# indianajohn/akaze-rust

Measured on AMD Instinct MI355X. Metric: Mpix/s through extract_features (4 oct x 4 sub), higher is better.
Workload: dtype f32

## Files before the change

akaze-rust_amd/csrc/akz_api.cpp:

```cpp
#include <cstdio>

#include "akz_ctx.hpp"

unsigned akz::host_cpu_share() {
    unsigned n = std::max(1u, std::thread::hardware_concurrency());
    cpu_set_t set;
    if (sched_getaffinity(0, sizeof(set), &set) == 0) n = std::max(1, CPU_COUNT(&set));
    if (FILE* f = fopen("/sys/fs/cgroup/cpu.max", "r")) {
        char q[32] = {0};
        long period = 0;
        if (fscanf(f, "%31s %ld", q, &period) == 2 && period > 0 && strcmp(q, "max") != 0)
            n = std::min<unsigned>(n, (unsigned)std::max(1L, atol(q) / period));
        fclose(f);
    }
    if (const char* e = std::getenv("LOCAL_WORLD_SIZE")) {
        const int ranks = atoi(e);
        if (ranks > 1) n = std::max(2u, n / (unsigned)ranks);
    }
    return std::max(1u, n);
}

int level_info_out(const std::vector<LevelPlan>& plan, uint64_t level, double* etime, double* esigma,
                          uint32_t* octave, uint32_t* sublevel, uint32_t* sigma_size, uint32_t* lw, uint32_t* lh,
                          uint32_t* det_sigma, uint64_t* n_tau, double* tau, uint64_t tau_cap) {
// ... 283 lines not shown
                return AKZ_ERR_INVALID_ARG;
            }
    c->settings.host_threads = threads;
    push_settings(c);
    for (akz_ctx* x : all) x->workers.reset();
    return AKZ_OK;
}
int akz_ctx_set_candidate_hint(akz_ctx* c, uint32_t per_image) {
    AKZ_TRY(bind(c));
    c->cand_cap_hint = std::max<uint32_t>(per_image, 16u);
    for (akz_ctx* l : c->lanes) l->cand_cap_hint = c->cand_cap_hint.load();
    return AKZ_OK;
}
int akz_ctx_set_match_mode(akz_ctx* c, int mode) {
    AKZ_TRY(bind(c));
    if (mode < 0 || mode > 3) return AKZ_ERR_INVALID_ARG;
    c->settings.match_mode = mode;
    push_settings(c);
    return AKZ_OK;
}
int akz_ctx_set_fed_mode(akz_ctx* c, int mode) {
    AKZ_TRY(bind(c));
    if (mode != 0 && mode != 2) return AKZ_ERR_INVALID_ARG;
    c->settings.fed_mode = mode;
    push_settings(c);
    return AKZ_OK;
}
const char* akz_fed_kernel_name(void) { return "k_level_march + k_fed_own"; }
int akz_debug_march_bands(int kind, uint32_t w, uint32_t h, uint32_t n, int half_width, int32_t* rows, uint32_t cap,
                          uint32_t* n_bands) {
    if (!n_bands || (cap && !rows) || kind < 0 || kind > 1 || w < 16 || h < 16 || n == 0 || half_width < 1 || half_width > 4)
        return AKZ_ERR_INVALID_ARG;
    *n_bands = launch::march_band_rows(kind, w, h, n, half_width, rows, cap);
    return AKZ_OK;
}
int akz_debug_detector_set_cells(int half_width, const uint32_t* w, const uint32_t* h, uint32_t n_entries, uint32_t n, int32_t* cells,
                                 uint32_t cap, int32_t* grids, uint32_t* n_workgroups) {
    if (!n_workgroups || !w || !h || !grids || (cap && !cells) || n_entries < 1 || n_entries > launch::detector_march_set_max() || n == 0 ||
        half_width < 1 || half_width > 4)
        return AKZ_ERR_INVALID_ARG;
    for (uint32_t e = 0; e < n_entries; ++e)
        if (w[e] < 4u * (uint32_t)half_width + 8u || h[e] < 4u * (uint32_t)half_width + 8u) return AKZ_ERR_INVALID_ARG;
    *n_workgroups = launch::detector_set_cells(half_width, w, h, n_entries, n, cells, cap, grids);
    return AKZ_OK;
}
const char* akz_detector_kernel_name(void) { return "detector (k_detector_march + k_detector_tiled)"; }
int akz_debug_set_schedule(akz_ctx* c, int key, int value) {
    if (!c || key < 0 || key >= SCHED_COUNT_) return AKZ_ERR_INVALID_ARG;
    AKZ_TRY(bind(c));
    CtxSettings& s = c->settings;
    s.sched[key] = value;
    if (key == SCHED_DET_BAND_ROWS || key == SCHED_LEVEL_BAND_ROWS)
        launch::march_min_band_rows(s.sched[SCHED_DET_BAND_ROWS], s.sched[SCHED_LEVEL_BAND_ROWS]);
    if (key == SCHED_DET_SETS) launch::detector_set_waves(value >= 11 && value <= 14 ? value - 10 : 0);
    if (key == SCHED_JOB_KPX) {
        s.big_px_sync = value > 0 ? (uint64_t)value * 1000u : gates::kBigPxSync;
        s.big_px_async = value > 0 ? (uint64_t)value * 1000u : gates::kBigPxAsync;
        s.lane_px = value > 0 ? (uint64_t)value * 1000u : gates::kLanePx;
    }
    push_settings(c);
    return AKZ_OK;
}
int akz_debug_placement_verdict(float spin_pair_ms, float tiny_pair_ms, float tiny_alone_ms, float spin_ms) {
    return akz::placement_verdict(spin_pair_ms, tiny_pair_ms, tiny_alone_ms, spin_ms);
}
int akz_debug_stream_placement(akz_ctx* c, int* info) {
// ... 161 lines not shown
```

akaze-rust_amd/csrc/akz_internal.hpp:

```cpp
#pragma once
#include <hip/hip_runtime.h>

#include <cstdint>
#include <functional>
#include <string>
#include <vector>

#include "../../include/akaze_hip.h"
#include "../../include/akaze_hip_debug.h"

namespace akz {

void set_error(const std::string& msg);
unsigned host_cpu_share();

using TrialsOnDevice = std::function<int(const float*, const float*, const float*, const float*, uint32_t, const uint32_t*, uint32_t,
                                         float, float, float*, int32_t*)>;
int remove_outliers_impl(const akz_keypoint* keypoints_0, uint64_t n0, const akz_keypoint* keypoints_1, uint64_t n1,
                         const akz_match* matches, uint64_t n_matches, uint64_t num_trials, float epsilon_model,
                         float epsilon_inlier, akz_match* out, uint64_t* n_out, const TrialsOnDevice& trials_on_device);

#define AKZ_HIP_TRY(expr)                                                                          \
    do {                                                                                           \
        hipError_t _e = (expr);                                                                    \
// ... 136 lines not shown
void contrast_max(hipStream_t s, const float* blurred, uint32_t w, uint32_t h, uint32_t n,
                  unsigned long long* d_hmax_bits);
void contrast_hist(hipStream_t s, const float* blurred, uint32_t w, uint32_t h, uint32_t n,
                   const unsigned long long* d_hmax_bits, uint32_t nbins, uint32_t* d_hist);
void contrast_final(hipStream_t s, const unsigned long long* d_hmax_bits, const uint32_t* d_hist, uint32_t nbins,
                    double percentile, uint32_t n, double* d_k);
bool blur_fused_supported(uint32_t ntaps);
void blur_fused_f32(hipStream_t s, const float* in, float* out, uint32_t w, uint32_t h, uint32_t n, const float* k,
                    uint32_t ntaps);
void blur_fused_u8(hipStream_t s, const uint8_t* in, float* out, uint32_t w, uint32_t h, uint32_t n, const float* k,
                   uint32_t ntaps);
void prep_fused(hipStream_t s, const float* prev, bool half, float* lt_out, float* lsmooth, float* lflow, uint32_t w,
                uint32_t h, uint32_t pw, uint32_t ph, uint32_t n, const float* g3, const double* d_k, uint32_t k_pow);
bool detector_fused_supported(uint32_t sigma);
void detector_fused(hipStream_t s, const float* lsmooth, uint32_t sigma, float* lx, float* ly, float* lxx, float* lyy,
                    float* lxy, float* ldet_out, uint32_t w, uint32_t h, uint32_t n);
bool detector_tiled_fused_supported(uint32_t sigma);
struct DetLevelDesc {
    const float* lsmooth;
    float *lx, *ly, *lxx, *lyy, *lxy, *ldet;
    uint32_t w, h, level;
    float border_m;
};
uint32_t detector_tiled_set_max();
void detector_tiled_set(hipStream_t s, uint32_t sigma, const DetLevelDesc* levels, uint32_t nlevels, uint32_t n, float thr,
                        Candidate* d_cand, uint32_t cap, uint32_t* d_count);
void detector_tiled_fused(hipStream_t s, const float* lsmooth, uint32_t sigma, float* lx, float* ly, float* lxx,
                          float* lyy, float* lxy, float* ldet_out, uint32_t w, uint32_t h, uint32_t n, uint32_t level,
                          float thr, float border_m, Candidate* d_cand, uint32_t cap, uint32_t* d_count);
bool blur5_stream_supported(uint32_t w, uint32_t h, uint32_t ntaps, bool is_u8);
void blur5_stream_u8(hipStream_t s, const uint8_t* in, float* out, uint32_t w, uint32_t h, uint32_t n, const float* k);
void blur5_stream_f32(hipStream_t s, const float* in, float* out, uint32_t w, uint32_t h, uint32_t n, const float* k);
uint32_t march_band_rows(int kind, uint32_t w, uint32_t h, uint32_t n, int S, int32_t* cs_ce, uint32_t cap);
bool blur5_march_supported(uint32_t w, uint32_t h, uint32_t ntaps);
void blur5_march_u8(hipStream_t s, const uint8_t* in, float* out, uint32_t w, uint32_t h, uint32_t n, const float* k);
void blur5_march_f32(hipStream_t s, const float* in, float* out, uint32_t w, uint32_t h, uint32_t n, const float* k);
bool contrast_march_supported(uint32_t w, uint32_t h, uint32_t ntaps, uint32_t nbins);
void contrast_march(hipStream_t s, const float* in, uint32_t w, uint32_t h, uint32_t n, const float* g3,
                    unsigned long long* d_hmax_bits, uint32_t nbins, uint32_t* d_hist, double* d_thr);
void contrast_thresholds(hipStream_t s, const unsigned long long* d_hmax_bits, uint32_t nbins, uint32_t n, double* d_thr);
bool contrast_stream_supported(uint32_t w, uint32_t h, uint32_t ntaps, uint32_t nbins);
void contrast_stream(hipStream_t s, const float* in, uint32_t w, uint32_t h, uint32_t n, const float* g3,
                     unsigned long long* d_hmax_bits, uint32_t nbins, uint32_t* d_hist, double* d_thr);
bool prep_stream_supported(uint32_t w, uint32_t h);
void prep_stream(hipStream_t s, const float* prev, bool half, float* lt_out, float* lsmooth, float* lflow, uint32_t w,
                 uint32_t h, uint32_t pw, uint32_t ph, uint32_t n, const float* g3, const double* d_k, uint32_t k_pow);
bool detector_march_supported(uint32_t sigma, uint32_t w, uint32_t h, float border_m, bool nms);
void detector_march(hipStream_t s, const float* lsmooth, uint32_t sigma, float* lx, float* ly, float* lxx, float* lyy,
                    float* lxy, float* ldet_out, uint32_t w, uint32_t h, uint32_t n, uint32_t level, float thr,
                    float border_m, Candidate* d_cand, uint32_t cap, uint32_t* d_count);
uint32_t detector_march_set_max();
void detector_march_set(hipStream_t s, uint32_t sigma, const DetLevelDesc* levels, uint32_t nlevels, uint32_t n, float thr,
                        Candidate* d_cand, uint32_t cap, uint32_t* d_count);
void detector_set_waves(int waves);
uint32_t detector_set_cells(int S, const uint32_t* w, const uint32_t* h, uint32_t nlv, uint32_t n, int32_t* cells, uint32_t cap,
                            int32_t* grids);
bool head_fused_supported(uint32_t w, uint32_t h, uint32_t ntaps0, uint32_t ntaps1);
void head_fused_u8(hipStream_t s, const uint8_t* in, float* lt0, float* blurred, float* gx, float* gy, uint32_t w, uint32_t h, uint32_t n,
                   const float* k5, const float* g3, unsigned long long* d_smax_bits, uint32_t* d_zero_word = nullptr);
void head_fused_f32(hipStream_t s, const float* in, float* lt0, float* blurred, float* gx, float* gy, uint32_t w, uint32_t h, uint32_t n,
                    const float* k5, const float* g3, unsigned long long* d_smax_bits, uint32_t* d_zero_word = nullptr);
void contrast_hist_final(hipStream_t s, const float* gx, const float* gy, uint32_t w, uint32_t h, uint32_t n, unsigned long long* d_smax_bits,
                         uint32_t nbins, uint32_t* d_hist, uint32_t* d_done, double percentile, double* d_k);
void flow_from_pair(hipStream_t s, const float* gx, const float* gy, float* lflow, uint32_t w, uint32_t h, uint32_t n, const double* d_k,
                    uint32_t k_pow);
void march_min_band_rows(int detector, int level);
// ... 198 lines not shown
```

akaze-rust_amd/csrc/akz_march.hip:

```cpp
#include <hip/hip_runtime.h>

#include <algorithm>
#include <cstdlib>
#include <type_traits>

#include "akz_internal.hpp"
#include "akz_pm_g2.hpp"

namespace akz {
namespace {

typedef float f2 __attribute__((ext_vector_type(2)));
typedef float f2u __attribute__((ext_vector_type(2), aligned(4)));

constexpr int MT = 256;
constexpr int MW = 2 * MT;
constexpr int HALO = 16;
constexpr int USE = MW - 2 * HALO;
constexpr int PAD = 8;
constexpr int ROW = MW + 2 * PAD;
constexpr int CBUF = 32;
#ifndef AKZ_MARCH_PF
#define AKZ_MARCH_PF 3
#endif

struct MarchGrid {
    int nstrips, nbands, band_rows;
    int edge_rows;
    int total;
};
#ifndef AKZ_MARCH_XCD
#define AKZ_MARCH_XCD 1
#endif
__device__ __forceinline__ int march_cell() {
#if AKZ_MARCH_XCD
    return (int)((blockIdx.x & 7u) * (gridDim.x >> 3) + (blockIdx.x >> 3));
#else
    return (int)blockIdx.x;
#endif
}
__host__ __device__ __forceinline__ void uniform_band_rows(const MarchGrid& g, int band, int S, int h, int* cs, int* ce) {
    *cs = S + band * g.band_rows;
    const int e = *cs + g.band_rows;
    *ce = e < h - S ? e : h - S;
}
__host__ __device__ __forceinline__ void level_band_rows(const MarchGrid& g, int band, int h, int* cs, int* ce) {
    *cs = 1 + (band == 0 ? 0 : g.edge_rows + (band - 1) * g.band_rows);
    const int e = *cs + (band == 0 ? g.edge_rows : g.band_rows);
    *ce = band == g.nbands - 1 ? h - 1 : (e < h - 1 ? e : h - 1);
}
struct MarchNms {
    unsigned level;
    float thr;
    int xlo, xhi, ylo, yhi;
    Candidate* cand;
    unsigned cap;
    unsigned* count;
};

constexpr int kDetSetMax = 4;
struct DetMarchEntry {
    const float* ls;
    float *lx, *ly, *ldet, *lxx, *lyy, *lxy;
    int w, h;
    MarchGrid g;
    unsigned level;
    int xlo, xhi, ylo, yhi;
    int first;
};
struct DetMarchSet {
    DetMarchEntry e[kDetSetMax];
};
#if defined(__HIP_DEVICE_COMPILE__)
#define AKZ_UNIFORM(x) __builtin_amdgcn_readfirstlane(x)
#else
#define AKZ_UNIFORM(x) (x)
#endif
__host__ __device__ __forceinline__ bool det_set_cell(const DetMarchSet& set, int wg, int nwg, DetMarchEntry* E, int* entry, int* img,
                                                      int* band, int* strip) {
#if AKZ_MARCH_XCD
    const int xcd = wg & 7, j = wg >> 3;
    (void)nwg;
// ... 351 lines not shown
    const int cell = march_cell();
    if (cell >= g.total) return;
    const int img = __builtin_amdgcn_readfirstlane(cell / per);
    const int rem = cell - img * per;
    const int band = __builtin_amdgcn_readfirstlane(rem / g.nstrips), strip = rem - band * g.nstrips;
    int cs, ce;
    level_band_rows(g, band, h, &cs, &ce);
    if (cs >= ce) return;
    const int lt0 = cs == 1 ? 0 : cs, lt1 = ce == h - 1 ? h : ce;

    const int X0 = strip * USE - HALO;
    const int p0 = (2 * tid + HALO) & (MW - 1);
    const bool inner = p0 >= HALO && p0 < MW - HALO;
    const Cols C = make_cols(X0 + p0, inner, w);
    const int i0 = PAD + clampi(clampi(C.x0, 1, w - 2) - X0, 0, MW - 1) - 1;
    const int i1 = PAD + clampi(clampi(C.x0 + 1, 1, w - 2) - X0, 0, MW - 1) - 1;
    const int wi = PAD + p0;
    const bool edge_h = __ballot(i0 != wi - 1 || i1 != wi) != 0ull;
    const bool hxn0 = C.x0 > 0, hxp0 = C.x0 + 1 < w, hxn1 = C.x0 + 1 > 0, hxp1 = C.x0 + 2 < w;
    const bool edge_col = __ballot(!(hxn0 && hxp0 && hxn1 && hxp1)) != 0ull;

    const size_t base = (size_t)img * (size_t)w * (size_t)h;
    const __amdgpu_buffer_rsrc_t in = HALF ? plane_rsrc(prev + (size_t)img * (size_t)pw * (size_t)ph, pw, ph) : plane_rsrc(prev + base, w, h);
    const __amdgpu_buffer_rsrc_t o_ls[1] = {plane_rsrc(lsmooth_out + base, w, h)};
    const __amdgpu_buffer_rsrc_t o_lf[1] = {plane_rsrc(lflow_out + base, w, h)};
    __amdgpu_buffer_rsrc_t o_lt[KEEPSTEP ? 2 : 1];
    o_lt[0] = plane_rsrc(lt_out + base, w, h);
    if (KEEPSTEP) o_lt[1] = plane_rsrc(lstep_out + base, w, h);
    const __amdgpu_buffer_rsrc_t(&o_ltc)[KEEPSTEP ? 2 : 1] = o_lt;
    const double kc = octave_contrast(d_k[img], k_pow);
    const double inverse_k = 1.0 / (kc * kc);

    const int v0 = lt0 - N - 2;
    const int T = (lt1 - lt0) + 2 * N + 6;
    struct Fed {
        f2 v;
        u4m top, bot;
    };
    auto feed = [&](int t) -> Fed {
        Fed f;
        const unsigned row = (unsigned)clampi(v0 + min(t, T - 1), 0, h - 1);
        if constexpr (HALF) {
            const unsigned ro = 2u * row * ((unsigned)pw * 4u);
            f.top = __builtin_amdgcn_raw_buffer_load_b128(in, (int)(2u * C.vo_ld), (int)ro, 0);
            f.bot = __builtin_amdgcn_raw_buffer_load_b128(in, (int)(2u * C.vo_ld), (int)(ro + (unsigned)pw * 4u), 0);
        } else {
            f.v = load_pair<ODDW>(in, row * ((unsigned)w * 4u), C);
        }
        return f;
    };
    auto pair_of = [&](const Fed& f) -> f2 {
        if constexpr (HALF) {
            float a = 0.0f, b = 0.0f;
            a = a + __uint_as_float(f.top.x); a = a + __uint_as_float(f.bot.x); a = a + __uint_as_float(f.top.y); a = a + __uint_as_float(f.bot.y);
            b = b + __uint_as_float(f.top.z); b = b + __uint_as_float(f.bot.z); b = b + __uint_as_float(f.top.w); b = b + __uint_as_float(f.bot.w);
            return f2{a / 4.0f, b / 4.0f};
        } else {
            return f.v;
        }
    };
    Fed q[4];
#pragma unroll
    for (int i = 0; i < PF; ++i) q[i] = feed(i);
    const f2 zero = {0.0f, 0.0f};
    f2 LP[8], CR[8];
    f2 GH[4], HM[4], HO[4];
    f2 SXW[4], SXE[4];
    f2 W[N > 1 ? N - 1 : 1][4];
#pragma unroll
    for (int i = 0; i < 8; ++i) LP[i] = CR[i] = zero;
#pragma unroll
    for (int i = 0; i < 4; ++i) {
        GH[i] = HM[i] = HO[i] = SXW[i] = SXE[i] = zero;
#pragma unroll
        for (int j = 0; j < (N > 1 ? N - 1 : 1); ++j) W[j][i] = zero;
    }
    f2 ls_c = zero, lf_c = zero, gh_c = zero;

    auto rows = [&](auto mid_tag) {
    constexpr bool MID = decltype(mid_tag)::value;
    for (int t0 = 0; t0 < T; t0 += 8) {
#pragma unroll
        for (int k = 0; k < 8; ++k) {
            const int t = t0 + k;
            {
                const int v = v0 + t;
                q[(k + PF) & 3] = feed(t + PF);
                float* const buf = &s_row[t & 1][0][0];
                LP[k & 7] = fix_pair(pair_of(q[k & 3]), C);
                *reinterpret_cast<f2*>(buf + 0 * ROW + wi) = LP[k & 7];
                *reinterpret_cast<f2*>(buf + 1 * ROW + wi) = ls_c;
                *reinterpret_cast<f2*>(buf + 2 * ROW + wi) = CR[(k - 5) & 7];
                *reinterpret_cast<f2*>(buf + 3 * ROW + wi) = LP[(k - 5) & 7];
#pragma unroll
                for (int s = 2; s <= N; ++s) *reinterpret_cast<f2*>(buf + (2 + s) * ROW + wi) = W[s - 2][(k - 1) & 3];
                __syncthreads();
                f2 gh = gh_c;
                if (MID || v <= h - 2) {
                    f2 a, b, c;
                    if (!rare(edge_h)) {
                        a = lds2(buf + wi - 1); b = LP[k & 7]; c = lds2(buf + wi + 1);
                    } else {
                        const float* r0 = buf + i0;
                        const float* r1 = buf + i1;
                        a = f2{r0[0], r1[0]}; b = f2{r0[1], r1[1]}; c = f2{r0[2], r1[2]};
                    }
                    gh = tap3(a, b, c, g0, g1, g2);
                }
                gh_c = gh;
                GH[k & 3] = gh;
                if (!MID && rare(v == 1)) GH[(k - 1) & 3] = gh;
                const int u = v - 1;
                f2 ls_n = ls_c;
                if (MID || u <= h - 2) ls_n = tap3(GH[(k - 2) & 3], GH[(k - 1) & 3], GH[k & 3], g0, g1, g2);
                {
                    const f2 o[1] = {ls_n};
                    if (MID) store_rows<1, ODDW>(o_ls, u, w, u >= cs && u < ce, C, o);
                    else store_filled<1, 1, ODDW>(o_ls, C, w, h, u, u >= cs && u < ce, o);
                }
                {
                    f2 a, b, c;
                    if (!rare(edge_h)) {
                        a = lds2(buf + ROW + wi - 1); b = ls_c; c = lds2(buf + ROW + wi + 1);
                    } else {
                        const float* r0 = buf + ROW + i0;
                        const float* r1 = buf + ROW + i1;
                        a = f2{r0[0], r1[0]}; b = f2{r0[1], r1[1]}; c = f2{r0[2], r1[2]};
                    }
                    HM[k & 3] = tap_main(a, b, c, kn, kwn);
                    HO[k & 3] = tap_off(a, c);
                }
                if (!MID && rare(u - 1 == 1)) {
                    HM[(k - 1) & 3] = HM[k & 3];
                    HO[(k - 1) & 3] = HO[k & 3];
                }
                const int c = v - 3;
                f2 lf_n = lf_c;
                if (MID || c <= h - 2) {
                    const f2 lx1 = tap_off(HM[(k - 2) & 3], HM[k & 3]);
                    const f2 ly1 = tap_main(HO[(k - 2) & 3], HO[(k - 1) & 3], HO[k & 3], kn, kwn);
                    lf_n = f2{pm_g2_px(lx1.x, ly1.x, inverse_k), pm_g2_px(lx1.y, ly1.y, inverse_k)};
                }
                CR[(k - 3) & 7] = lf_n;
                if (!MID && rare(c == 1)) CR[(k - 4) & 7] = lf_n;
                {
                    const f2 o[1] = {lf_n};
                    if (MID) store_rows<1, ODDW>(o_lf, c, w, c >= cs && c < ce, C, o);
                    else store_filled<1, 1, ODDW>(o_lf, C, w, h, c, c >= cs && c < ce, o);
                }
                {
                    const float* cr = buf + 2 * ROW + wi;
                    const f2 cc = CR[(k - 5) & 7];
                    SXW[k & 3] = lds2(cr - 1) + cc;
                    SXE[k & 3] = cc + lds2(cr + 1);
                }
                f2 lnew = zero, st = zero;
#pragma unroll
                for (int s = 1; s <= N; ++s) {
                    const int r = v - 4 - s;
                    f2 Lm, Lc, Lp;
                    if (s == 1) {
                        Lm = LP[(k - 6) & 7]; Lc = LP[(k - 5) & 7]; Lp = LP[(k - 4) & 7];
                    } else {
                        W[s - 2][k & 3] = lnew;
                        Lm = W[s - 2][(k - 2) & 3]; Lc = W[s - 2][(k - 1) & 3]; Lp = lnew;
                    }
                    const float* lr = buf + (2 + s) * ROW + wi;
                    const f2 Lw = lds2(lr - 1), Le = lds2(lr + 1);
                    const f2 cN = CR[(k - 5 - s) & 7], cC = CR[(k - 4 - s) & 7], cS = CR[(k - 3 - s) & 7];
                    const f2 SU = cN + cC, SV = cC + cS;
                    const f2 XFW = SXW[(k - (s - 1)) & 3] * (Lc - Lw);
                    const f2 XFE = SXE[(k - (s - 1)) & 3] * (Le - Lc);
                    f2 tx;
                    if (!edge_col) {
                        tx = XFE - XFW;
                    } else {
                        tx.x = hxp0 ? (hxn0 ? XFE.x - XFW.x : XFE.x) : -XFW.x;
                        tx.y = hxp1 ? (hxn1 ? XFE.y - XFW.y : XFE.y) : -XFW.y;
                    }
                    f2 tt;
                    if (MID || r + 1 < h) {
                        tt = tx + SV * (Lp - Lc);
                        if (MID || r > 0) tt = tt - SU * (Lc - Lm);
                    } else {
                        tt = tx + SU * (Lm - Lc);
                    }
                    st = ht.half_tau[s - 1] * tt;
                    lnew = Lc + st;
                }
                {
                    const int r = v - 4 - N;
                    {
                        f2 o[KEEPSTEP ? 2 : 1];
                        o[0] = lnew;
                        if constexpr (KEEPSTEP) o[1] = st;
                        const f2(&oc)[KEEPSTEP ? 2 : 1] = o;
                        store_rows<KEEPSTEP ? 2 : 1, ODDW>(o_ltc, r, w, r >= lt0 && r < lt1, C, oc);
                    }
                }
                ls_c = ls_n;
                lf_c = lf_n;
            }
        }
    }
    };
    const int v_last = v0 + ((T + 7) & ~7) - 1;
    if (v0 >= N + 5 && v_last <= h - 2) rows(std::true_type{});
    else rows(std::false_type{});
}

struct ContrastMarchArgs {
    unsigned long long* hmax_bits;
    unsigned* hist;
    unsigned nbins;
    const double* thr;
};
constexpr int CM_COPIES = 2;
template <int MODE, bool ODDW>
__global__ void __launch_bounds__(MT, 8)
k_contrast_march(const float* __restrict__ in_plane, int w, int h, MarchGrid g, float g0, float g1, float g2, float kn,
                 float kwn, ContrastMarchArgs ca) {
    constexpr int PF = 2;
    __shared__ __attribute__((aligned(16))) float s_row[2][2][ROW];
    extern __shared__ __attribute__((aligned(16))) unsigned s_chist[];
    const int tid = threadIdx.x, lane = tid & 63, wv = tid >> 6;
    const int per = g.nbands * g.nstrips;
    const int cell = march_cell();
    if (cell >= g.total) return;
    const int img = __builtin_amdgcn_readfirstlane(cell / per);
    const int rem = cell - img * per;
    const int band = __builtin_amdgcn_readfirstlane(rem / g.nstrips), strip = rem - band * g.nstrips;
    int cs, ce;
    level_band_rows(g, band, h, &cs, &ce);
    if (cs >= ce) return;
    const int lt0 = cs == 1 ? 0 : cs, lt1 = ce == h - 1 ? h : ce;

    const int X0 = strip * USE - HALO;
    const int p0 = (2 * tid + HALO) & (MW - 1);
    const bool inner = p0 >= HALO && p0 < MW - HALO;
// ... 472 lines not shown
    const MarchGrid mg = plan_level_march(w, h, n, &gr, 8, g_head_min_rows > 0 ? g_head_min_rows : 32);
    if (w & 1u)
        hipLaunchKernelGGL((k_contrast_march<1, true>), gr, dim3(MT), 0, s, in, (int)w, (int)h, mg, g3[0], g3[1], g3[2], m.wgt[0], m.wgt[1], ca);
    else
        hipLaunchKernelGGL((k_contrast_march<1, false>), gr, dim3(MT), 0, s, in, (int)w, (int)h, mg, g3[0], g3[1], g3[2], m.wgt[0], m.wgt[1], ca);
    contrast_thresholds(s, d_hmax_bits, nbins, n, d_thr);
    const size_t lds = ((size_t)(MT / 64) * CM_COPIES * nbins) * sizeof(unsigned) + (size_t)(nbins + 1) * sizeof(double);
    if (w & 1u)
        hipLaunchKernelGGL((k_contrast_march<2, true>), gr, dim3(MT), lds, s, in, (int)w, (int)h, mg, g3[0], g3[1], g3[2], m.wgt[0], m.wgt[1], ca);
    else
        hipLaunchKernelGGL((k_contrast_march<2, false>), gr, dim3(MT), lds, s, in, (int)w, (int)h, mg, g3[0], g3[1], g3[2], m.wgt[0], m.wgt[1], ca);
}

#ifndef AKZ_LVL_FILL
#define AKZ_LVL_FILL 3
#endif
static int level_min_band_rows(uint32_t w, uint32_t h, uint32_t n) {
    if (g_lvl_min_rows > 0) return g_lvl_min_rows;
    return (uint64_t)w * h * n < (48u << 20) ? 20 : 64;
}
uint32_t march_band_rows(int kind, uint32_t w, uint32_t h, uint32_t n, int S, int32_t* cs_ce, uint32_t cap) {
    dim3 gr;
    const MarchGrid g = kind == 1 ? plan_level_march(w, h, n, &gr, AKZ_LVL_FILL, level_min_band_rows(w, h, n)) : plan_march(w, h, n, S, &gr);
    for (int b = 0; b < g.nbands && (uint32_t)b < cap; ++b) {
        int cs, ce;
        if (kind == 1) level_band_rows(g, b, (int)h, &cs, &ce);
        else uniform_band_rows(g, b, S, (int)h, &cs, &ce);
        cs_ce[2 * b] = cs;
        cs_ce[2 * b + 1] = ce;
    }
    return (uint32_t)g.nbands;
}

bool level_march_supported(uint32_t w, uint32_t h) { return w >= 16 && h >= 16 && (uint64_t)w * h <= (1ull << 28); }

template <int NS, bool KEEPSTEP>
static void launch_level_march(hipStream_t s, dim3 gr, const MarchGrid& mg, const float* prev, float* lsmooth, float* lflow,
                               float* lt_out, float* lstep, uint32_t w, uint32_t h, const float* g3, const Taps& m,
                               const double* d_k, uint32_t k_pow, const LevelTaus& ht, uint32_t pw, uint32_t ph) {
    if constexpr (NS == 4) {
        if (pw) {
            hipLaunchKernelGGL((k_level_march<NS, KEEPSTEP, false, true>), gr, dim3(MT), 0, s, prev, lsmooth, lflow, lt_out, lstep, (int)w,
                               (int)h, mg, g3[0], g3[1], g3[2], m.wgt[0], m.wgt[1], d_k, k_pow, ht, (int)pw, (int)ph);
            return;
        }
    }
    if (w & 1u)
        hipLaunchKernelGGL((k_level_march<NS, KEEPSTEP, true>), gr, dim3(MT), 0, s, prev, lsmooth, lflow, lt_out, lstep, (int)w,
                           (int)h, mg, g3[0], g3[1], g3[2], m.wgt[0], m.wgt[1], d_k, k_pow, ht);
    else
        hipLaunchKernelGGL((k_level_march<NS, KEEPSTEP, false>), gr, dim3(MT), 0, s, prev, lsmooth, lflow, lt_out, lstep, (int)w,
                           (int)h, mg, g3[0], g3[1], g3[2], m.wgt[0], m.wgt[1], d_k, k_pow, ht);
}
#define AKZ_LEVEL(NS)                                                                                                        \
    case NS: {                                                                                                               \
        if (lstep) launch_level_march<NS, true>(s, gr, mg, prev, lsmooth, lflow, lt_out, lstep, w, h, g3, m, d_k, k_pow, ht, pw, ph);  \
        else launch_level_march<NS, false>(s, gr, mg, prev, lsmooth, lflow, lt_out, lstep, w, h, g3, m, d_k, k_pow, ht, pw, ph);       \
    } break;

bool level_march_half_supported(uint32_t w, uint32_t h, uint32_t pw, uint32_t ph, uint32_t n_steps) {
    return n_steps == 4 && (pw & 3u) == 0 && (w & 1u) == 0 && w == pw / 2 && h == ph / 2 && (uint64_t)pw * ph <= (1ull << 28);
}
void level_march(hipStream_t s, const float* prev, float* lsmooth, float* lflow, float* lt_out, float* lstep, uint32_t w,
                 uint32_t h, uint32_t n, const float* g3, const double* d_k, uint32_t k_pow, const float* half_taus,
                 uint32_t n_steps, uint32_t pw, uint32_t ph) {
    const Taps m = taps_scharr_main(1);
// ... 14 lines not shown
```

akaze-rust_amd/python/akaze_amd.py:

```python
import ctypes as C
import os

import numpy as np

_PKG = os.path.dirname(os.path.dirname(os.path.abspath(__file__)))
LIB_PATH = os.environ.get("AKAZE_HIP_LIB") or os.path.join(_PKG, "libakaze_hip.so")

AKZ_KEEP_ALL_PLANES = 1
AKZ_NO_HOST_DESCRIPTORS = 2
AKZ_NO_DETECT = 4
AKZ_INPUT_READY = 8
AKZ_ERR_BUFFER = -7

PLANES = ["Lt", "Lsmooth", "Lx", "Ly", "Lxx", "Lyy", "Lxy", "Lflow", "Lstep", "Ldet"]

FRAME_GRAY8, FRAME_RGB8, FRAME_BGR8, FRAME_RGBA8, FRAME_BGRA8, FRAME_RGB8_PLANAR = range(6)
KR_FRAME_LUMA = 12
KR_MASK_CANDIDATES = 13


class AkazeError(RuntimeError):
    def __init__(self, status, msg):
        super().__init__(f"akaze_hip status {status}: {msg}")
        self.status = status
# ... 244 lines not shown
        "akz_random_color": ([vp], i32),
        "akz_draw_circle": ([vp, u32, u32, C.c_float, C.c_float, vp, C.c_float], i32),
        "akz_draw_line": ([vp, u32, u32, C.c_float, C.c_float, C.c_float, C.c_float, vp, C.c_float], i32),
        "akz_job_abandon": ([vp], i32),
        "akz_result_free": ([vp], i32),
        "akz_result_num_images": ([vp, pu64], i32),
        "akz_result_counts": ([vp, u64, pu64, pu64, pu64], i32),
        "akz_result_keypoints": ([vp, u64, vp], i32),
        "akz_result_descriptors": ([vp, u64, vp], i32),
        "akz_result_device_descriptors": ([vp, u64, C.POINTER(vp), pu64], i32),
        "akz_result_contrast": ([vp, u64, pf64], i32),
        "akz_result_copy_device_descriptors": ([vp, vp, u64, pu64], i32),
        "akz_result_level_info": ([vp, u64, pf64, pf64, pu32, pu32, pu32, pu32, pu32, pu64, pf64, u64], i32),
        "akz_fetch_plane": ([vp, u64, u64, i32, vp, pu64], i32),
        "akz_fetch_pyramid": ([vp, u64, vp, u64, pu64], i32),
        "akz_result_device_plane": ([vp, u64, u64, i32, C.POINTER(vp)], i32),
        "akz_descriptor_match": ([vp, vp, u64, vp, u64, u64, u64, f64, vp, pu64], i32),
        "akz_descriptor_match_device": ([vp, vp, u64, vp, u64, u64, f64, vp, vp], i32),
        "akz_ctx_graph_probe": ([vp, vp, u32, u32, u32, C.POINTER(Config), u32, u32, pf64, pf64, pu64], i32),
        "akz_debug_march_bands": ([i32, u32, u32, u32, i32, C.POINTER(i32), u32, pu32], i32),
        "akz_ctx_set_lanes": ([vp, u32], i32),
        "akz_ctx_set_eager_finish": ([vp, i32], i32),
        "akz_fed_kernel_name": ([], C.c_char_p),
        "akz_ctx_set_host_threads": ([vp, u32], i32),
        "akz_debug_set_match_chunks": ([vp, u32, u32], i32),
        "akz_debug_set_host_sort": ([vp, i32], i32),
        "akz_debug_set_alloc_fill": ([vp, i32], i32),
        "akz_debug_audit_scratch": ([vp, vp, u32, pu32], i32),
        "akz_debug_resource_counts": ([pu64], i32),
        "akz_debug_set_select": ([vp, i32], i32),
        "akz_debug_select_info": ([vp, C.POINTER(C.c_int)], i32),
        "akz_debug_set_schedule": ([vp, i32, i32], i32),
        "akz_debug_detector_set_cells": ([i32, pu32, pu32, u32, u32, C.POINTER(i32), u32, C.POINTER(i32), pu32], i32),
        "akz_debug_stream_placement": ([vp, C.POINTER(i32)], i32),
        "akz_detector_kernel_name": ([], C.c_char_p),
        "akz_remove_outliers": ([vp, u64, vp, u64, vp, u64, u64, C.c_float, C.c_float, vp, pu64], i32),
        "akz_estimate_fundamental_matrix": ([vp, u64, vp, u64, vp, C.c_float, fp, C.POINTER(i32)], i32),
        "akz_match_features": ([vp, vp, u64, vp, u64, vp, u64, vp, u64, u64, f64, u64, C.c_float, vp, pu64], i32),
        "akz_match_features_pairs": ([vp, vp, u64, vp, u64, u64, f64, u64, C.c_float, vp, pu64], i32),
        "akz_debug_ransac_samples": ([u64, u64, u64, u64, pu64], i32),
        "akz_debug_ransac_samples_k": ([u64, u64, u64, u64, i32, pu64], i32),
        "akz_estimate_homography": ([vp, u64, vp, u64, vp, C.c_float, fp, C.POINTER(i32)], i32),
        "akz_remove_outliers_homography": ([vp, u64, vp, u64, vp, u64, u64, C.c_float, C.c_float, vp, pu64, fp, C.POINTER(i32)], i32),
        "akz_match_features_homography": ([vp, vp, u64, vp, u64, vp, u64, vp, u64, u64, f64, u64, C.c_float, vp, pu64, fp,
                                           C.POINTER(i32)], i32),
        "akz_match_features_homography_pairs": ([vp, vp, u64, vp, u64, u64, f64, u64, C.c_float, vp, pu64, fp, C.POINTER(i32)], i32),
        "akz_refine_homography": ([vp, u64, vp, u64, vp, u64, fp, C.c_float, C.c_uint32, vp, pu64, fp, C.POINTER(C.c_uint32)], i32),
        "akz_match_features_homography_refined": ([vp, vp, u64, vp, u64, vp, u64, vp, u64, u64, f64, u64, C.c_float, C.c_uint32, vp, pu64,
                                                   fp, C.POINTER(i32), C.POINTER(C.c_uint32)], i32),
        "akz_match_features_homography_refined_pairs": ([vp, vp, u64, vp, u64, u64, f64, u64, C.c_float, C.c_uint32, vp, pu64, fp,
                                                         C.POINTER(i32), C.POINTER(C.c_uint32)], i32),
        "akz_match_features_homography_refined_guided": ([vp, vp, u64, vp, u64, vp, u64, vp, u64, u64, f64, u64, C.c_float, C.c_uint32,
                                                          C.c_float, f64, vp, pu64, fp, C.POINTER(i32), C.POINTER(C.c_uint32)], i32),
        "akz_match_features_homography_refined_guided_pairs": ([vp, vp, u64, vp, u64, u64, f64, u64, C.c_float, C.c_uint32, C.c_float, f64,
                                                                vp, pu64, fp, C.POINTER(i32), C.POINTER(C.c_uint32)], i32),
        "akz_descriptor_match_guided_host": ([vp, u64, vp, u64, vp, u64, vp, u64, u64, i32, fp, C.c_float, u64, f64, vp, pu64], i32),
        "akz_descriptor_match_guided": ([vp, vp, u64, vp, u64, vp, u64, vp, u64, u64, i32, fp, C.c_float, u64, f64, vp, pu64], i32),
        "akz_descriptor_match_guided_pairs": ([vp, vp, u64, vp, u64, u64, i32, fp, C.c_float, u64, f64, vp, pu64], i32),
        "akz_match_features_homography_guided": ([vp, vp, u64, vp, u64, vp, u64, vp, u64, u64, f64, u64, C.c_float, C.c_float, f64, vp,
                                                  pu64, fp, C.POINTER(i32)], i32),
        "akz_match_features_homography_guided_pairs": ([vp, vp, u64, vp, u64, u64, f64, u64, C.c_float, C.c_float, f64, vp, pu64, fp,
                                                        C.POINTER(i32)], i32),
        "akz_remove_outliers_fundamental": ([vp, u64, vp, u64, vp, u64, u64, C.c_float, C.c_float, vp, pu64, fp, C.POINTER(i32)], i32),
        "akz_refine_fundamental_matrix": ([vp, u64, vp, u64, vp, u64, fp, C.c_float, C.c_uint32, vp, pu64, fp, C.POINTER(C.c_uint32)], i32),
        "akz_match_features_fundamental": ([vp, vp, u64, vp, u64, vp, u64, vp, u64, u64, f64, u64, C.c_float, vp, pu64, fp,
                                            C.POINTER(i32)], i32),
# ... 1963 lines not shown
```

include/akaze_hip_debug.h:

```cpp
#ifndef AKAZE_HIP_DEBUG_H
#define AKAZE_HIP_DEBUG_H
#include "akaze_hip.h"
#ifdef __cplusplus
extern "C" {
#endif

int akz_ctx_graph_probe(akz_ctx* ctx, const uint8_t* d_imgs, uint32_t w, uint32_t h, uint32_t n, const akz_config* cfg,
                        uint32_t flags, uint32_t reps, double* ms_graph, double* ms_plain, uint64_t* graph_nodes);
int akz_debug_march_bands(int kind, uint32_t w, uint32_t h, uint32_t n, int half_width, int32_t* rows, uint32_t cap,
                          uint32_t* n_bands);
int akz_debug_detector_set_cells(int half_width, const uint32_t* w, const uint32_t* h, uint32_t n_entries, uint32_t n, int32_t* cells,
                                 uint32_t cap, int32_t* grids, uint32_t* n_workgroups);
const char* akz_fed_kernel_name(void);
const char* akz_detector_kernel_name(void);
int akz_debug_set_match_chunks(akz_ctx* ctx, uint32_t pair_chunks, uint32_t set_chunks);
int akz_debug_match_tile_rows(uint32_t* rows);
int akz_debug_set_knn_chunks(akz_ctx* ctx, uint32_t chunks);
int akz_debug_set_schedule(akz_ctx* ctx, int key, int value);
int akz_debug_stream_placement(akz_ctx* ctx, int* info);
int akz_debug_placement_verdict(float spin_pair_ms, float tiny_pair_ms, float tiny_alone_ms, float spin_ms);
int akz_debug_device_libm(akz_ctx* ctx, int* available, int* last_job);
int akz_debug_set_device_libm(akz_ctx* ctx, int mode);
int akz_debug_libm_eval(akz_ctx* ctx, const float* d_a, const float* d_b, float* d_out3, uint64_t n, int fma);
typedef struct akz_gate {
    const char* name;
    double value;
    const char* unit;
    const char* meaning;
} akz_gate;
int akz_debug_gates(const akz_gate** rows, uint64_t* n);
int akz_ctx_calibrate_gates(akz_ctx* ctx, uint64_t* sync_px, uint64_t* async_px, double* ms);
enum { AKZ_KR_LEVEL_MARCH = 1, AKZ_KR_FED_OWN = 2, AKZ_KR_OCTAVE_RESIDENT = 3, AKZ_KR_DETECTOR_TILED = 4, AKZ_KR_DETECTOR_MARCH = 5,
       AKZ_KR_JPEG_IDCT = 6, AKZ_KR_JPEG_LUMA = 7, AKZ_KR_JPEG_COPY = 8, AKZ_KR_SORT_ROWS = 9, AKZ_KR_SORT_BUCKETS = 10,
       AKZ_KR_SORT_RADIX = 11, AKZ_KR_FRAME_LUMA = 12, AKZ_KR_MASK_CANDIDATES = 13 };
typedef struct akz_kernel_row {
    uint32_t stage, kind, param, w, h, n;
    uint64_t launches, px, px_steps;
    double ms;
} akz_kernel_row;
int akz_debug_kernel_rows(akz_ctx* ctx, akz_kernel_row* out, uint32_t cap, uint32_t* n_rows, int reset);
int akz_debug_rcp_f64_to_f32(akz_ctx* ctx, const double* d_x, float* d_out, uint64_t n);
int akz_debug_set_host_sort(akz_ctx* ctx, int on);
int akz_debug_set_select(akz_ctx* ctx, int mode);
int akz_debug_select_info(akz_ctx* ctx, int* info);

// ... 31 lines not shown
```

Baseline: 15110.

## Split level-march row loop into fill, steady and drain groups skipping dead stages

Restructures the row-marching loop of the level march kernel into fill groups, a steady plain loop and drain groups. Each pipeline stage (Gaussian, Scharr, flow, x-sum, FED steps) now runs only inside its computed live window of time steps. This removes wasted arithmetic during pipeline warm-up and past the end, including the padding rows from rounding T up to a multiple of eight. The cost is more code instantiations and register pressure, plus a new debug API exposing the windows.

```diff
diff --git a/akaze-rust_amd/csrc/akz_api.cpp b/akaze-rust_amd/csrc/akz_api.cpp
--- a/akaze-rust_amd/csrc/akz_api.cpp
+++ b/akaze-rust_amd/csrc/akz_api.cpp
@@ -339,6 +339,11 @@
     if (!n_bands || (cap && !rows) || kind < 0 || kind > 1 || w < 16 || h < 16 || n == 0 || half_width < 1 || half_width > 4)
         return AKZ_ERR_INVALID_ARG;
     *n_bands = launch::march_band_rows(kind, w, h, n, half_width, rows, cap);
+    return AKZ_OK;
+}
+int akz_debug_level_windows(uint32_t rows, uint32_t n_steps, int32_t* out) {
+    if (!out || rows < 1 || rows > (1u << 28) || n_steps < 1 || n_steps > 4) return AKZ_ERR_INVALID_ARG;
+    launch::level_march_windows(rows, n_steps, out);
     return AKZ_OK;
 }
 int akz_debug_detector_set_cells(int half_width, const uint32_t* w, const uint32_t* h, uint32_t n_entries, uint32_t n, int32_t* cells,
diff --git a/akaze-rust_amd/csrc/akz_internal.hpp b/akaze-rust_amd/csrc/akz_internal.hpp
--- a/akaze-rust_amd/csrc/akz_internal.hpp
+++ b/akaze-rust_amd/csrc/akz_internal.hpp
@@ -192,6 +192,7 @@
 void blur5_stream_u8(hipStream_t s, const uint8_t* in, float* out, uint32_t w, uint32_t h, uint32_t n, const float* k);
 void blur5_stream_f32(hipStream_t s, const float* in, float* out, uint32_t w, uint32_t h, uint32_t n, const float* k);
 uint32_t march_band_rows(int kind, uint32_t w, uint32_t h, uint32_t n, int S, int32_t* cs_ce, uint32_t cap);
+void level_march_windows(uint32_t rows, uint32_t n_steps, int32_t* out21);
 bool blur5_march_supported(uint32_t w, uint32_t h, uint32_t ntaps);
 void blur5_march_u8(hipStream_t s, const uint8_t* in, float* out, uint32_t w, uint32_t h, uint32_t n, const float* k);
 void blur5_march_f32(hipStream_t s, const float* in, float* out, uint32_t w, uint32_t h, uint32_t n, const float* k);
diff --git a/akaze-rust_amd/csrc/akz_march.hip b/akaze-rust_amd/csrc/akz_march.hip
--- a/akaze-rust_amd/csrc/akz_march.hip
+++ b/akaze-rust_amd/csrc/akz_march.hip
@@ -48,6 +48,23 @@
     *cs = 1 + (band == 0 ? 0 : g.edge_rows + (band - 1) * g.band_rows);
     const int e = *cs + (band == 0 ? g.edge_rows : g.band_rows);
     *ce = band == g.nbands - 1 ? h - 1 : (e < h - 1 ? e : h - 1);
+}
+struct LevelWindows {
+    int T;
+    int hgauss[2], vgauss[2], hscharr[2], flow[2], xsum[2], fed[4][2], full[2];
+};
+__host__ __device__ __forceinline__ LevelWindows level_windows(int rows, int N) {
+    LevelWindows W;
+    const int T = rows + 2 * N + 6;
+    W.T = T;
+    W.hgauss[0] = 0, W.hgauss[1] = T - 2;
+    W.vgauss[0] = 2, W.vgauss[1] = T - 2;
+    W.hscharr[0] = 3, W.hscharr[1] = T - 1;
+    W.flow[0] = 5, W.flow[1] = T - 1;
+    W.xsum[0] = 8, W.xsum[1] = T;
+    for (int s = 1; s <= 4; ++s) W.fed[s - 1][0] = s <= N ? 6 + 2 * s : T, W.fed[s - 1][1] = T;
+    W.full[0] = 6 + 2 * N, W.full[1] = T - 2;
+    return W;
 }
 struct MarchNms {
     unsigned level;
@@ -465,7 +482,8 @@
     const double inverse_k = 1.0 / (kc * kc);
 
     const int v0 = lt0 - N - 2;
-    const int T = (lt1 - lt0) + 2 * N + 6;
+    const LevelWindows lw = level_windows(lt1 - lt0, N);
+    const int T = lw.T;
     struct Fed {
         f2 v;
         u4m top, bot;
@@ -510,9 +528,19 @@
     }
     f2 ls_c = zero, lf_c = zero, gh_c = zero;
 
-    auto rows = [&](auto mid_tag) {
+    constexpr int PLAIN = 0, FILL = 1, DRAIN = 2;
+    auto before_end = [](int t, int end) -> bool {
+        if (t < end) {
+            asm volatile("");
+            return true;
+        }
+        return false;
+    };
+    auto group = [&](auto mid_tag, auto mode_tag, const int t0) __attribute__((always_inline)) {
     constexpr bool MID = decltype(mid_tag)::value;
-    for (int t0 = 0; t0 < T; t0 += 8) {
+    constexpr int MODE = decltype(mode_tag)::value;
+    auto live = [&](const int (&win)[2], int t) -> bool { return MODE == PLAIN || (MODE == FILL ? t >= win[0] : before_end(t, win[1])); };
+    {
 #pragma unroll
         for (int k = 0; k < 8; ++k) {
             const int t = t0 + k;
@@ -529,7 +557,7 @@
                 for (int s = 2; s <= N; ++s) *reinterpret_cast<f2*>(buf + (2 + s) * ROW + wi) = W[s - 2][(k - 1) & 3];
                 __syncthreads();
                 f2 gh = gh_c;
-                if (MID || v <= h - 2) {
+                if ((live(lw.hgauss, t)) && (MID || v <= h - 2)) {
                     f2 a, b, c;
                     if (!rare(edge_h)) {
                         a = lds2(buf + wi - 1); b = LP[k & 7]; c = lds2(buf + wi + 1);
@@ -545,31 +573,34 @@
                 if (!MID && rare(v == 1)) GH[(k - 1) & 3] = gh;
                 const int u = v - 1;
                 f2 ls_n = ls_c;
-                if (MID || u <= h - 2) ls_n = tap3(GH[(k - 2) & 3], GH[(k - 1) & 3], GH[k & 3], g0, g1, g2);
+                if ((live(lw.vgauss, t)) && (MID || u <= h - 2))
+                    ls_n = tap3(GH[(k - 2) & 3], GH[(k - 1) & 3], GH[k & 3], g0, g1, g2);
                 {
                     const f2 o[1] = {ls_n};
                     if (MID) store_rows<1, ODDW>(o_ls, u, w, u >= cs && u < ce, C, o);
                     else store_filled<1, 1, ODDW>(o_ls, C, w, h, u, u >= cs && u < ce, o);
                 }
-                {
-                    f2 a, b, c;
-                    if (!rare(edge_h)) {
-                        a = lds2(buf + ROW + wi - 1); b = ls_c; c = lds2(buf + ROW + wi + 1);
-                    } else {
-                        const float* r0 = buf + ROW + i0;
-                        const float* r1 = buf + ROW + i1;
-                        a = f2{r0[0], r1[0]}; b = f2{r0[1], r1[1]}; c = f2{r0[2], r1[2]};
+                if (live(lw.hscharr, t)) {
+                    {
+                        f2 a, b, c;
+                        if (!rare(edge_h)) {
+                            a = lds2(buf + ROW + wi - 1); b = ls_c; c = lds2(buf + ROW + wi + 1);
+                        } else {
+                            const float* r0 = buf + ROW + i0;
+                            const float* r1 = buf + ROW + i1;
+                            a = f2{r0[0], r1[0]}; b = f2{r0[1], r1[1]}; c = f2{r0[2], r1[2]};
+                        }
+                        HM[k & 3] = tap_main(a, b, c, kn, kwn);
+                        HO[k & 3] = tap_off(a, c);
                     }
-                    HM[k & 3] = tap_main(a, b, c, kn, kwn);
-                    HO[k & 3] = tap_off(a, c);
-                }
-                if (!MID && rare(u - 1 == 1)) {
-                    HM[(k - 1) & 3] = HM[k & 3];
-                    HO[(k - 1) & 3] = HO[k & 3];
+                    if (!MID && rare(u - 1 == 1)) {
+                        HM[(k - 1) & 3] = HM[k & 3];
+                        HO[(k - 1) & 3] = HO[k & 3];
+                    }
                 }
                 const int c = v - 3;
                 f2 lf_n = lf_c;
-                if (MID || c <= h - 2) {
+                if ((live(lw.flow, t)) && (MID || c <= h - 2)) {
                     const f2 lx1 = tap_off(HM[(k - 2) & 3], HM[k & 3]);
                     const f2 ly1 = tap_main(HO[(k - 2) & 3], HO[(k - 1) & 3], HO[k & 3], kn, kwn);
                     lf_n = f2{pm_g2_px(lx1.x, ly1.x, inverse_k), pm_g2_px(lx1.y, ly1.y, inverse_k)};
@@ -581,7 +612,7 @@
                     if (MID) store_rows<1, ODDW>(o_lf, c, w, c >= cs && c < ce, C, o);
                     else store_filled<1, 1, ODDW>(o_lf, C, w, h, c, c >= cs && c < ce, o);
                 }
-                {
+                if (live(lw.xsum, t)) {
                     const float* cr = buf + 2 * ROW + wi;
                     const f2 cc = CR[(k - 5) & 7];
                     SXW[k & 3] = lds2(cr - 1) + cc;
@@ -591,11 +622,12 @@
 #pragma unroll
                 for (int s = 1; s <= N; ++s) {
                     const int r = v - 4 - s;
+                    if (s > 1) W[s - 2][k & 3] = lnew;
+                    if (live(lw.fed[s - 1], t)) {
                     f2 Lm, Lc, Lp;
                     if (s == 1) {
                         Lm = LP[(k - 6) & 7]; Lc = LP[(k - 5) & 7]; Lp = LP[(k - 4) & 7];
                     } else {
-                        W[s - 2][k & 3] = lnew;
                         Lm = W[s - 2][(k - 2) & 3]; Lc = W[s - 2][(k - 1) & 3]; Lp = lnew;
                     }
                     const float* lr = buf + (2 + s) * ROW + wi;
@@ -620,6 +652,7 @@
                     }
                     st = ht.half_tau[s - 1] * tt;
                     lnew = Lc + st;
+                    }
                 }
                 {
                     const int r = v - 4 - N;
@@ -637,7 +670,17 @@
         }
     }
     };
-    const int v_last = v0 + ((T + 7) & ~7) - 1;
+    auto rows = [&](auto mid_tag) {
+        group(mid_tag, std::integral_constant<int, FILL>{}, 0);
+        if constexpr (N > 1) {
+            if (T > 8) group(mid_tag, std::integral_constant<int, FILL>{}, 8);
+        }
+        int t0 = N > 1 ? 16 : 8;
+        static_assert(6 + 2 * N <= (N > 1 ? 16 : 8), "fill groups");
+        for (; t0 + 8 <= lw.full[1]; t0 += 8) group(mid_tag, std::integral_constant<int, PLAIN>{}, t0);
+        for (; t0 < T; t0 += 8) group(mid_tag, std::integral_constant<int, DRAIN>{}, t0);
+    };
+    const int v_last = v0 + T - 1;
     if (v0 >= N + 5 && v_last <= h - 2) rows(std::true_type{});
     else rows(std::false_type{});
 }
@@ -1176,6 +1219,13 @@
     return (uint32_t)g.nbands;
 }
 
+void level_march_windows(uint32_t rows, uint32_t n_steps, int32_t* out) {
+    const LevelWindows W = level_windows((int)rows, (int)n_steps);
+    const int* wins[10] = {W.hgauss, W.vgauss, W.hscharr, W.flow, W.xsum, W.fed[0], W.fed[1], W.fed[2], W.fed[3], W.full};
+    out[0] = W.T;
+    for (int i = 0; i < 10; ++i) out[1 + 2 * i] = wins[i][0], out[2 + 2 * i] = wins[i][1];
+}
+
 bool level_march_supported(uint32_t w, uint32_t h) { return w >= 16 && h >= 16 && (uint64_t)w * h <= (1ull << 28); }
 
 template <int NS, bool KEEPSTEP>
diff --git a/akaze-rust_amd/python/akaze_amd.py b/akaze-rust_amd/python/akaze_amd.py
--- a/akaze-rust_amd/python/akaze_amd.py
+++ b/akaze-rust_amd/python/akaze_amd.py
@@ -300,6 +300,7 @@
         "akz_debug_select_info": ([vp, C.POINTER(C.c_int)], i32),
         "akz_debug_set_schedule": ([vp, i32, i32], i32),
         "akz_debug_detector_set_cells": ([i32, pu32, pu32, u32, u32, C.POINTER(i32), u32, C.POINTER(i32), pu32], i32),
+        "akz_debug_level_windows": ([u32, u32, C.POINTER(i32)], i32),
         "akz_debug_stream_placement": ([vp, C.POINTER(i32)], i32),
         "akz_detector_kernel_name": ([], C.c_char_p),
         "akz_remove_outliers": ([vp, u64, vp, u64, vp, u64, u64, C.c_float, C.c_float, vp, pu64], i32),
diff --git a/include/akaze_hip_debug.h b/include/akaze_hip_debug.h
--- a/include/akaze_hip_debug.h
+++ b/include/akaze_hip_debug.h
@@ -11,6 +11,7 @@
                           uint32_t* n_bands);
 int akz_debug_detector_set_cells(int half_width, const uint32_t* w, const uint32_t* h, uint32_t n_entries, uint32_t n, int32_t* cells,
                                  uint32_t cap, int32_t* grids, uint32_t* n_workgroups);
+int akz_debug_level_windows(uint32_t rows, uint32_t n_steps, int32_t* out);
 const char* akz_fed_kernel_name(void);
 const char* akz_detector_kernel_name(void);
 int akz_debug_set_match_chunks(akz_ctx* ctx, uint32_t pair_chunks, uint32_t set_chunks);
```

Result: slower. 14850 (-1.7%).
